# Aidan900/ppa-nbody-collisions

Hardware: AMD Instinct MI355X
Metric: body-pair-interactions/sec at N=262144 (higher is better)
Workload: dtype f32; 1 GPU; BASELINE.json configs[3] (the metric's configuration): N=262144 bodies, fp32, radii 0, reference initial condition (seed 1024), literal reference step semantics, 98 steps; bodies_after=262110, parallelism=single GPU

## Files before the change

ppa-nbody-collisions_amd/csrc/nbody_kernels.hpp:

```cpp
#pragma once
#include <hip/hip_runtime.h>
#include <stdint.h>
#include <type_traits>

#include "nbody.h"
#include "nbody_partition.h"

#pragma clang fp contract(off)

namespace nbk {

constexpr int kTile = 128;
constexpr int kWave = 64;

template <typename T> struct Rec;
template <> struct alignas(16) Rec<float> { float x, y, m, r; };
template <> struct alignas(32) Rec<double> { double x, y, m, r; };
template <typename T> struct alignas(2 * sizeof(T)) Vec2 { T x, y; };

struct alignas(16) RecPadded {
    double x, y, m, r, pad0, pad1;
    __device__ __forceinline__ RecPadded& operator=(const Rec<double>& o) { x = o.x; y = o.y; m = o.m; r = o.r; return *this; }
    __device__ __forceinline__ operator Rec<double>() const { return Rec<double>{x, y, m, r}; }
};
// ... 474 lines not shown
    __shared__ RecPadded tile_all[2][2][2 * kTile];                                                          \
    __shared__ int tile_bad_all[2][2][kTile / kWave];                                                        \
    __shared__ int tile_rnz_all[2][2][kTile / kWave];                                                        \
    RecPadded(&tile)[2][2 * kTile] = tile_all[threadIdx.x / kTile];                                          \
    int(&tile_bad)[2][kTile / kWave] = tile_bad_all[threadIdx.x / kTile];                                    \
    int(&tile_rnz)[2][kTile / kWave] = tile_rnz_all[threadIdx.x / kTile];
#define NB_V3_LANE const int lane = threadIdx.x % kTile;
#define NB_V3_WG const int wg = blockIdx.x * 2 + threadIdx.x / kTile;
#define NB_V3_BATCH 8
#define NB_V3_CONSTANTS constexpr int K = 1;
#define NB_V3_RANGE const int N = meta->n, lo = meta->lo, cnt = meta->cnt, step = meta->step;
#define NB_V3_REC(j) J[j]
#define NB_V3_VEL(i) Vown[i - lo]
#define NB_V3_PUT(q, i, out, vout) S_J[q] = out; S_V[q] = vout;
#define NB_V3_KEEP(q, i, a, v) S_J[q] = Rec<T>{a.xi, a.yi, a.mi, a.ri}; S_V[q] = v;
#define NB_V3_COUNT(pairs)                                                                                   \
    for (int sh = kWave / 2; sh > 0; sh >>= 1) pairs += __shfl_down(pairs, sh, kWave);                      \
    if ((lane & (kWave - 1)) == 0 && pairs) atomicAdd(&ctr->pairs, pairs);
#include "nbody_forces_v3.inc"
#undef NB_V3_ROTATE_PRIORITY
#undef NB_V3_TILE_REC
#undef NB_V3_REAL
#undef NB_V3_SIGNATURE
#undef NB_V3_LDS
#undef NB_V3_LANE
#undef NB_V3_WG
#undef NB_V3_BATCH
#undef NB_V3_CONSTANTS
#undef NB_V3_RANGE
#undef NB_V3_REC
#undef NB_V3_VEL
#undef NB_V3_PUT
#undef NB_V3_KEEP
#undef NB_V3_COUNT

#ifndef NBK_TEMPLATES_ONLY
#define NB_V3_REAL float
#define NB_V3_SIGNATURE                                                                                      \
    __global__ __launch_bounds__(2 * kTile, 4) void ref_layout_forces_v3_f32(                                \
        void* bodyData, float* __restrict__ updM, float* __restrict__ updR, const int N, StepParams<float> p)
#define NB_V3_LDS                                                                                            \
    __shared__ Rec<T> tile_all[2][2][2 * kTile];                                                             \
    __shared__ int tile_bad_all[2][2][kTile / kWave];                                                        \
    __shared__ int tile_rnz_all[2][2][kTile / kWave];                                                        \
    Rec<T>(&tile)[2][2 * kTile] = tile_all[threadIdx.x / kTile];                                             \
    int(&tile_bad)[2][kTile / kWave] = tile_bad_all[threadIdx.x / kTile];                                    \
    int(&tile_rnz)[2][kTile / kWave] = tile_rnz_all[threadIdx.x / kTile];
#define NB_V3_LANE const int lane = threadIdx.x % kTile;
#define NB_V3_WG const int wg = blockIdx.x * 2 + threadIdx.x / kTile;
#define NB_V3_BATCH 8
#define NB_V3_CONSTANTS                                                                                      \
    constexpr int K = 1;                                                                                     \
    constexpr bool kLog = false;
#define NB_V3_RANGE                                                                                          \
    constexpr int lo = 0, step = 0, ev_cap = 0;                                                              \
    const int cnt = N;                                                                                       \
    Event* const ev = nullptr;                                                                               \
    Counters* const ctr = nullptr;                                                                           \
    const Vec2<float>* __restrict__ P = reinterpret_cast<const Vec2<float>*>(bodyData);        \
    Vec2<float>* __restrict__ V = reinterpret_cast<Vec2<float>*>(bodyData) + N;                              \
    const float* __restrict__ M = reinterpret_cast<const float*>(V + N);                                     \
    const float* __restrict__ R = M + N;
#define NB_V3_REC(j) Rec<float>{P[j].x, P[j].y, M[j], R[j]}
#define NB_V3_VEL(i) V[i]
#define NB_V3_PUT(q, i, out, vout) (void)q; updM[i] = out.m; updR[i] = out.r; V[i] = vout;
#define NB_V3_KEEP(q, i, a, v) (void)q;
#define NB_V3_COUNT(pairs) (void)pairs;
#include "nbody_forces_v3.inc"
#undef NB_V3_REAL
#undef NB_V3_SIGNATURE
#undef NB_V3_LDS
#undef NB_V3_LANE
#undef NB_V3_WG
#undef NB_V3_BATCH
#undef NB_V3_CONSTANTS
#undef NB_V3_RANGE
#undef NB_V3_REC
#undef NB_V3_VEL
#undef NB_V3_PUT
#undef NB_V3_KEEP
#undef NB_V3_COUNT
#endif

typedef __attribute__((address_space(3))) void* LdsPtr;
typedef int Int4 __attribute__((ext_vector_type(4)));
typedef float Float2 __attribute__((ext_vector_type(2)));
typedef float Float4 __attribute__((ext_vector_type(4)));
typedef volatile __attribute__((address_space(3))) Int4* LdsInt4Ptr;
typedef volatile __attribute__((address_space(3))) Float4* LdsFloat4Ptr;

constexpr int kRingDeadSeq = 0x40000000;
constexpr unsigned long long kIndexError = 1ull << 32;
__device__ __forceinline__ int batch_checked_count(int n, int stride) { return (n < 0 || n > stride) ? -1 : n; }

#pragma clang diagnostic push
#pragma clang diagnostic ignored "-Winline-asm"
__device__ __forceinline__ void load_to_lds_b32(const void* base, unsigned byte_offset, unsigned lds_dst) {
    asm volatile("s_mov_b32 m0, %0\n\ts_nop 0\n\tglobal_load_lds_dword %1, %2"
                 ::"s"(lds_dst), "v"(byte_offset), "s"(base) : "memory", "m0");
}
#pragma clang diagnostic pop
__device__ __forceinline__ unsigned lds_offset_of(const void* p) { return (unsigned)(unsigned long long)(LdsPtr)p; }

struct RingArgs {
    const Vec2<float>* Vown;
    Rec<float>* S_J;
    Vec2<float>* S_V;
    const Meta* meta;
    StepParams<float> p;
    Event* ev;
    int ev_cap;
    Counters* ctr;
    const float* tile_rmax;
    const float* Jt;
    int cap_own;
    int n_tiles;
    unsigned* q_head;
    unsigned long long* q_done;
    unsigned long long* q_state;
    unsigned q_launch;
    int q_rings;
    int q_whole;
    int q_seg_tiles;
};
typedef __attribute__((address_space(1))) unsigned* GlobalU32Ptr;
typedef __attribute__((address_space(1))) unsigned long long* GlobalU64Ptr;
typedef volatile __attribute__((address_space(3))) long long* LdsI64Ptr;
template <typename A>
__device__ __forceinline__ A ring_late_arg(unsigned byte_offset) {
#if defined(__HIP_DEVICE_COMPILE__)
    typedef const __attribute__((address_space(4))) char* KernargBytes;
    const KernargBytes ka = (KernargBytes)__builtin_amdgcn_kernarg_segment_ptr();
    asm volatile("" : "+s"(byte_offset));
    return *(const __attribute__((address_space(4))) A*)(ka + byte_offset);
#else
    (void)byte_offset;
    return A{};
#endif
}
#define NB_RING_LATE(field) \
    ring_late_arg<decltype(((const RingArgs*)nullptr)->field)>((unsigned)__builtin_offsetof(RingArgs, field))

template <bool kLog, int kW, int kT, int kSleep, bool kProbe, int kRings, bool kQueue = false>
__global__ __launch_bounds__(kRings * kW * kWave) __attribute__((amdgpu_waves_per_eu(4, 4)))
void forces_ring_f32(const RingArgs args) {
    typedef float T;
    const Meta* __restrict__ const meta = args.meta;
    const float* __restrict__ const tile_rmax = args.tile_rmax;
    const float* __restrict__ const Jt = args.Jt;
    typedef Pair<float>::type V2;
    static_assert(kTile % kT == 0 && kT % 8 == 0 && kT <= kWave, "turn length");
    constexpr int kTurnsPerTile = kTile / kT;
    constexpr bool kSolo = kW == 1;
    static_assert(kSolo || kW % kTurnsPerTile == 0, "a wave's successive turns are whole tiles apart");
    constexpr int kTilesPerRound = kW / kTurnsPerTile;
    constexpr int kWin = kWave + kT;
    static_assert(kSolo ? kRings == 16 && !kProbe : kRings == 1 || kRings == 2 || kRings == 4, "rings (64 bodies each) per workgroup");
    static_assert(!kQueue || kSolo || kW == kTurnsPerTile, "persistent form: an item is whole tiles and a wave keeps its part of every tile");
    __shared__ float win_all[kRings][kW][2][4][kWin];
    __shared__ Int4 hand_all[kSolo ? 1 : kRings][kWave];
    __shared__ Float4 hand_m_all[kRings][kWave];
    __shared__ int solo_done_all[kSolo ? kRings : 1];
    __shared__ long long item_all[kQueue && !kSolo ? kRings : 1][2];
    const int N = meta->n, lo = meta->lo, cnt = meta->cnt;
    const bool all_bounded = (meta->summary & kSummaryUnbounded) == 0, any_radius = (meta->summary & kSummaryRadius) != 0;
    const bool nan_screen = meta->summary == 0;
    const int tid = threadIdx.x;
    const int wv = __builtin_amdgcn_readfirstlane(tid / kWave);
    const int ring = wv / kW;
    const int w = wv % kW;
    const int l = tid % kWave;
    const int wg = blockIdx.x;
    const int slot = wg * kRings + ring;
    float(&win)[kW][2][4][kWin] = win_all[ring];
    Int4(&hand)[kWave] = hand_all[kSolo ? 0 : ring];
    Float4(&hand_m)[kWave] = hand_m_all[ring];
    const int nb = N < kTile ? 1 : N / kTile;
    const bool lit = args.p.literal != 0;
    const int ntiles = lit ? nb : (N + kTile - 1) / kTile;
    const int nturns = ntiles * kTurnsPerTile;
    const int q_spin_limit = kQueue ? __builtin_amdgcn_readfirstlane(args.p.spin_limit) : 0;
    bool dead = false;
    int timeouts = 0;
    unsigned long long pr_eval = 0, pr_wait = 0, pr_chain = 0, pr_check = 0, pr_polls = 0, pr_turns = 0, pr_t0 = 0, pr_r0 = 0;
    int seq_base = 0;
    int claims = 0;
    Int4 solo_h = Int4{0, 0, 0, 0};
    typedef volatile __attribute__((address_space(3))) int* LdsIntPtr;
    int solo_done = 0;
    if (kSolo) *(LdsIntPtr)&solo_done_all[wv] = 0;
    if (kQueue && !kSolo) {
        if (w == 0) {
            *(LdsInt4Ptr)&hand[l] = Int4{0, 0, 0, 0};
            if (l < 2) *(LdsI64Ptr)&item_all[ring][l] = 0ll;
        }
        __syncthreads();
        if (kProbe) { pr_t0 = __builtin_readcyclecounter(); pr_r0 = wall_clock64(); }
    }
    for (;;) {
        int ring_g = slot;
        int tau_lo = 0, tau_hi = nturns, seg = 0;
        if (kQueue) {
            const LdsI64Ptr entry = (LdsI64Ptr)&item_all[ring][claims & 1];
            claims += 1;
            const int q_whole = NB_RING_LATE(q_whole), q_cut = NB_RING_LATE(q_rings) - q_whole;
            const int seg_tiles = NB_RING_LATE(q_seg_tiles);
            const int nseg = (ntiles + seg_tiles - 1) / seg_tiles;
            auto decode = [&](int k) -> int {
                if ((long long)k >= q_whole + (long long)q_cut * nseg) return 0;
                ring_g = k; seg = 0; tau_lo = 0; tau_hi = nturns;
                if (k >= q_whole) {
                    seg = (k - q_whole) / q_cut;
                    ring_g = q_whole + (k - q_whole) % q_cut;
                    tau_lo = seg * seg_tiles * kTurnsPerTile;
                    tau_hi = tau_lo + seg_tiles * kTurnsPerTile < nturns ? tau_lo + seg_tiles * kTurnsPerTile : nturns;
                }
                const long long first = (long long)(lo / kTile + ring_g / 2) * kTile + (ring_g % 2) * kWave;
                return first >= (long long)lo + cnt ? 1 : 2;
            };
            auto decode_solo = [&](int k) -> int {
                const int rings = q_whole + q_cut;
                const int lead = q_whole < ntiles ? q_whole : ntiles;
                const int solo_nseg = 1 + (ntiles - lead + seg_tiles - 1) / seg_tiles;
                if ((long long)k >= (long long)rings * solo_nseg) return 0;
                seg = k / rings;
                ring_g = k - seg * rings;
                tau_lo = seg == 0 ? 0 : (lead + (seg - 1) * seg_tiles) * kTurnsPerTile;
                tau_hi = seg == 0 ? lead * kTurnsPerTile : tau_lo + seg_tiles * kTurnsPerTile;
                tau_hi = tau_hi < nturns ? tau_hi : nturns;
                const long long first = (long long)(lo / kTile + ring_g / 2) * kTile + (ring_g % 2) * kWave;
                return first >= (long long)lo + cnt ? 1 : 2;
            };
            int k = 0x7fffffff, what = 0;
            if (w == 0) {
                do {
                    unsigned drawn = 0;
                    if (l == 0) drawn = __hip_atomic_fetch_add((GlobalU32Ptr)NB_RING_LATE(q_head), 1u, __ATOMIC_RELAXED, __HIP_MEMORY_SCOPE_AGENT);
                    k = __builtin_amdgcn_readfirstlane((int)(drawn < 0x7fffffffu ? drawn : 0x7fffffffu));
                    what = kSolo ? decode_solo(k) : decode(k);
                } while (what == 1);
                if (!kSolo && l == 0) *entry = ((long long)claims << 32) | (long long)k;
            } else {
                for (int spins = 0;;) {
                    const long long e = *entry;
                    if (__builtin_amdgcn_readfirstlane((int)(e >> 32)) == claims) { k = __builtin_amdgcn_readfirstlane((int)e); break; }
                    if (++spins > q_spin_limit) { timeouts += 1; break; }
                    if (kSleep > 0) __builtin_amdgcn_s_sleep(kSleep);
                }
                what = decode(k);
            }
            if (what != 2) break;
        }
        const int half = ring_g % 2;
        const int b = lo / kTile + ring_g / 2;
        const int t0 = half * kWave;
        const int t = t0 + l;
        const long long blk0 = (long long)b * kTile;

        const bool mine = blk0 + t >= lo && blk0 + t < (long long)lo + cnt;
        const bool active = mine && blk0 + t < N && (!lit || blk0 + t < (long long)nb * kTile);
        auto body_index64 = [&]() -> long long {
            int lane = l;
            asm volatile("" : "+v"(lane));
            return blk0 + t0 + lane;
        };
        T xi = 0, yi = 0, ri = 0;
        {
            T mi = 0;
            if (mine) {
                const long long i64 = blk0 + t;
                const int i = (int)(i64 < 0x7fffffff ? i64 : 0x7fffffff);
                const float* me = Jt + (size_t)(i / kTile) * (4 * kTile) + (i % kTile);
                xi = me[0]; yi = me[kTile]; mi = me[2 * kTile]; ri = me[3 * kTile];
            }
            asm volatile("" : "+v"(xi), "+v"(yi), "+v"(mi), "+v"(ri));
            if (kQueue) {
                if (w == 0) {
                    Int4 h0 = Int4{0, 0, kSolo ? 0 : seq_base, 0};
                    Float4 m0 = Float4{mi, ri, mi, 0.0f};
                    bool late = false;
                    for (int spins = 0; !kSolo;) {
                        const Int4 h = *(LdsInt4Ptr)&hand[l];
                        if (__ballot(h.z < seq_base) == 0ull) break;
                        if (++spins > q_spin_limit) { late = true; break; }
                        if (kSleep > 0) __builtin_amdgcn_s_sleep(kSleep);
                    }
                    if (tau_lo > 0) {
                        const GlobalU64Ptr done = (GlobalU64Ptr)NB_RING_LATE(q_done) + ring_g;
                        const unsigned long long want = ((unsigned long long)NB_RING_LATE(q_launch) << 32) | (unsigned)seg;
                        for (int spins = 0; !late;) {
                            const unsigned long long have = __hip_atomic_load(done, __ATOMIC_RELAXED, __HIP_MEMORY_SCOPE_AGENT);
                            if (__ballot(have < want) == 0ull) break;
                            if (++spins > q_spin_limit) { late = true; break; }
                            if (kSleep > 0) __builtin_amdgcn_s_sleep(kSleep);
                        }
                        const GlobalU64Ptr rs = (GlobalU64Ptr)NB_RING_LATE(q_state) + (size_t)ring_g * (4 * kWave) + l;
                        const unsigned long long s0 = __hip_atomic_load(rs, __ATOMIC_RELAXED, __HIP_MEMORY_SCOPE_AGENT);
                        const unsigned long long s1 = __hip_atomic_load(rs + kWave, __ATOMIC_RELAXED, __HIP_MEMORY_SCOPE_AGENT);
                        const unsigned long long s2 = __hip_atomic_load(rs + 2 * kWave, __ATOMIC_RELAXED, __HIP_MEMORY_SCOPE_AGENT);
                        const unsigned long long s3 = __hip_atomic_load(rs + 3 * kWave, __ATOMIC_RELAXED, __HIP_MEMORY_SCOPE_AGENT);
                        h0 = Int4{(int)(unsigned)s0, (int)(unsigned)(s0 >> 32),
                                  (int)(unsigned)s1 >= kRingDeadSeq ? kRingDeadSeq : kSolo ? 0 : seq_base, (int)(unsigned)(s1 >> 32)};
                        m0 = Float4{__uint_as_float((unsigned)s2), __uint_as_float((unsigned)(s2 >> 32)), __uint_as_float((unsigned)s3), 0.0f};
                    }
                    if (late) { timeouts += 1; dead = true; }
                    if (kSolo && __ballot(h0.z >= kRingDeadSeq) != 0ull) dead = true;
                    if (dead) {
                        h0 = Int4{(int)0x7fc00000, (int)0x7fc00000, kRingDeadSeq, 0};
                        m0.x = m0.y = __builtin_nanf("");
                    }
                    *(LdsFloat4Ptr)&hand_m[l] = m0;
                    if (kSolo) solo_h = h0;
                    else *(LdsInt4Ptr)&hand[l] = h0;
                }
            } else if (w == 0) {
                if (kSolo) solo_h = Int4{0, 0, 0, 0};
                else *(LdsInt4Ptr)&hand[l] = Int4{0, 0, 0, 0};
                *(LdsFloat4Ptr)&hand_m[l] = Float4{mi, ri, mi, 0.0f};
            }
        }
        const int spin_limit = __builtin_amdgcn_readfirstlane(args.p.spin_limit);
        const bool lane_ok = !active || ((abs_(xi) < kCoordBound) && (abs_(yi) < kCoordBound));
        const bool wave_ok = __ballot(!lane_ok) == 0ull;
        int pairs_rare = 0;
        const LdsInt4Ptr hand_l = (LdsInt4Ptr)&hand[l];
        const LdsFloat4Ptr hand_m_l = (LdsFloat4Ptr)&hand_m[l];
        if (!kQueue) {
            if (!kSolo) __syncthreads();
            if (blk0 + t0 >= (long long)lo + cnt) return;
        }
        typedef const volatile __attribute__((address_space(3))) int* LdsSeqPtr;
        auto seq_of_ring_of = [&](int lane) -> LdsSeqPtr { return (LdsSeqPtr)&hand_all[lane % kRings][0] + 2; };
        LdsSeqPtr seq_look_kept = seq_of_ring_of(kLog ? 0 : l);
        if (!kLog && !kSolo && kRings > 1) asm volatile("" : "+v"(seq_look_kept));
        auto any_ring_ahead = [&]() -> bool {
            if (kLog) {
                int ahead = *seq_of_ring_of(ring + 1);
                if (kRings == 4) {
                    const int o2 = *seq_of_ring_of(ring + 2), o3 = *seq_of_ring_of(ring + 3);
                    ahead = ahead > o2 ? ahead : o2;
                    ahead = ahead > o3 ? ahead : o3;
                }
                return *seq_of_ring_of(ring) < ahead;
            }
            const int theirs = *seq_look_kept;
            const int ours = ((LdsSeqPtr)hand_l)[2];
            return __ballot(ours < theirs) != 0ull;
        };
        if (kProbe && !kQueue) { pr_t0 = __builtin_readcyclecounter(); pr_r0 = wall_clock64(); }

        auto tile_start_slow = [&](int kk) -> long long {
            if (!lit) return (long long)kk * kTile;
            return (blk0 % N + (long long)kk * kTile) % N;
        };
        typedef typename std::conditional<kLog, long long, unsigned>::type Idx;
        const Idx Nu = (Idx)N;
        auto round_on = [&](Idx st) -> Idx {
            st += kTilesPerRound * kTile;
            if (lit) while (st >= Nu) st -= Nu;
            return st;
        };
        auto tile_on = [&](Idx st) -> Idx {
            st += kTile;
            if (lit) while (st >= Nu) st -= Nu;
            return st;
        };
        auto tile_len = [&](int kk, Idx st) -> int {
            if (lit) return (kk == nb - 1) ? N % (kTile + 1) : kTile;
            if (kLog) return (Nu - st) < kTile ? (int)(Nu - st) : kTile;
            const int rest = (int)(Nu - st);
            return rest < kTile ? rest : kTile;
        };
        auto turn_kind = [&](int tau, Idx st) -> int {
            if (tau >= tau_hi) return 0;
            return tile_len(tau / kTurnsPerTile, st) == kTile ? 1 : 2;
        };
        auto fast_tile = [&](int kk) -> bool { return lit || kk != b; };
        const int wbase0 = lit ? t0 : 0;
        const int nwin = lit ? (kWave + kT - 1) : kT;
        auto entry_bytes_of = [&](int lane) -> unsigned {
            return ((unsigned)(wbase0 + (w % kTurnsPerTile) * kT + lane) & (kTile - 1)) * (unsigned)sizeof(T);
        };
        unsigned entry0_kept = kLog ? 0u : entry_bytes_of(l);
        if (!kLog) asm volatile("" : "+v"(entry0_kept));
        auto window_offset = [&](Idx st, unsigned e) -> unsigned {
            const unsigned src = (unsigned)st + e;
            const unsigned wrapped = src - (unsigned)N;
            const unsigned idx = src < wrapped ? src : wrapped;
            return ((idx / kTile) * (4u * kTile) + (idx % kTile)) * (unsigned)sizeof(T);
        };
        auto issue_entries = [&](unsigned tile_byte, unsigned byte_offset, unsigned base, unsigned comp_bytes) {
            unsigned long long plane = kTile * sizeof(T);
            asm volatile("" : "+s"(plane));
            if (kLog) {
                const unsigned long long last = (unsigned long long)tile_byte + byte_offset + 3 * kTile * sizeof(T) + sizeof(T);
                if (last > (unsigned long long)NB_RING_LATE(n_tiles) * (4 * kTile * sizeof(T))) {
                    atomicAdd(&NB_RING_LATE(ctr)->errors, kIndexError);
                    return;
                }
            }
            const char* const src = (const char*)Jt + tile_byte;
            load_to_lds_b32(src, byte_offset, base);
            load_to_lds_b32(src + plane, byte_offset, base + comp_bytes);
            load_to_lds_b32(src + 2 * plane, byte_offset, base + 2 * comp_bytes);
            if (any_radius) load_to_lds_b32(src + 3 * plane, byte_offset, base + 3 * comp_bytes);
        };
        auto solo_quarter = [&](int tau) -> unsigned { return (unsigned)(tau % kTurnsPerTile) * (kT * (unsigned)sizeof(T)); };
        auto issue_window = [&](Idx st, int buf, unsigned quarter_bytes) {
            const unsigned base = __builtin_amdgcn_readfirstlane(lds_offset_of(&win[w][buf][0][0]));
            if (kLog) {
                int lane = l;
                asm volatile("" : "+v"(lane));
                const unsigned e0 = (unsigned)(wbase0 + (w % kTurnsPerTile) * kT + lane + (kSolo ? quarter_bytes / (unsigned)sizeof(T) : 0u)) & (kTile - 1);
                const unsigned e1 = e0 ^ kWave;
                if (((unsigned)st & (kTile - 1)) == 0u && st + kTile <= Nu) {
                    const unsigned tile_byte = ((unsigned)st / kTile) * (4u * kTile * (unsigned)sizeof(T));
                    if (l < nwin) issue_entries(tile_byte, e0 * (unsigned)sizeof(T), base, kWin * (unsigned)sizeof(T));
                    if (l + kWave < nwin) issue_entries(tile_byte, e1 * (unsigned)sizeof(T), base + kWave * (unsigned)sizeof(T), kWin * (unsigned)sizeof(T));
                } else {
                    if (l < nwin) issue_entries(0u, window_offset(st, e0), base, kWin * (unsigned)sizeof(T));
                    if (l + kWave < nwin) issue_entries(0u, window_offset(st, e1), base + kWave * (unsigned)sizeof(T), kWin * (unsigned)sizeof(T));
                }
                return;
            }
            const unsigned entry0_bytes = kSolo ? (entry0_kept + quarter_bytes) & (kTile * (unsigned)sizeof(T) - 1u) : entry0_kept;
            const unsigned entry1_bytes = entry0_bytes ^ (kWave * (unsigned)sizeof(T));
            if (((unsigned)st & (kTile - 1)) == 0u && st + kTile <= Nu) {
                const unsigned tile_byte = ((unsigned)st / kTile) * (4u * kTile * (unsigned)sizeof(T));
                if (l < nwin) issue_entries(tile_byte, entry0_bytes, base, kWin * (unsigned)sizeof(T));
                if (l + kWave < nwin) issue_entries(tile_byte, entry1_bytes, base + kWave * (unsigned)sizeof(T), kWin * (unsigned)sizeof(T));
            } else {
                if (l < nwin) issue_entries(0u, window_offset(st, entry0_bytes / (unsigned)sizeof(T)), base, kWin * (unsigned)sizeof(T));
                if (l + kWave < nwin) issue_entries(0u, window_offset(st, entry1_bytes / (unsigned)sizeof(T)), base + kWave * (unsigned)sizeof(T), kWin * (unsigned)sizeof(T));
            }
        };
        static_assert(2 * kWin >= kTile, "a whole tile fits the two window buffers");
        float* const whole = &win[w][0][0][0];
        auto issue_truncated = [&](Idx st, int L) {
            const unsigned base = __builtin_amdgcn_readfirstlane(lds_offset_of(whole));
            if (l < L) issue_entries(0u, window_offset(st, (unsigned)l), base, kTile * (unsigned)sizeof(T));
            if (l + kWave < L) issue_entries(0u, window_offset(st, (unsigned)(l + kWave)), base + kWave * (unsigned)sizeof(T), kTile * (unsigned)sizeof(T));
        };
        auto window_record = [&](const float* comp0, int stride, int idx) -> Rec<T> {
            return Rec<T>{comp0[idx], comp0[stride + idx], comp0[2 * stride + idx], any_radius ? comp0[3 * stride + idx] : 0.0f};
        };
        auto window_rmax = [&](Idx st) -> float {
            if (!any_radius) return 0.0f;
            const int ta = __builtin_amdgcn_readfirstlane((int)(st / kTile));
            if (kLog && (ta < 0 || ta + 1 >= NB_RING_LATE(n_tiles))) {
                if (l == 0) atomicAdd(&NB_RING_LATE(ctr)->errors, kIndexError);
                return __builtin_inff();
            }
            const float ra = tile_rmax[ta], rb = tile_rmax[ta + 1];
            const float rw = (st + kTile > Nu) ? tile_rmax[0] : 0.0f;
            const float rab = ra > rb ? ra : rb;
            return rab > rw ? rab : rw;
        };
        struct WindowState { bool fast; float rmax; };
        auto check_window = [&](int kind, int kk, int buf, Idx st_w) -> WindowState {
            if (kind != 1) return WindowState{false, 0.0f};
            asm volatile("s_waitcnt vmcnt(0)" ::: "memory");
            __builtin_amdgcn_wave_barrier();
            if (all_bounded) return WindowState{wave_ok && fast_tile(kk), window_rmax(st_w)};
            Rec<T> r0{0, 0, 0, 0}, r1{0, 0, 0, 0};
            if (l < nwin) r0 = window_record(&win[w][buf][0][0], kWin, l);
            if (l + kWave < nwin) r1 = window_record(&win[w][buf][0][0], kWin, l + kWave);
            const bool bad0 = !((abs_(r0.x) < kCoordBound) && (abs_(r0.y) < kCoordBound));
            const bool bad1 = !((abs_(r1.x) < kCoordBound) && (abs_(r1.y) < kCoordBound));
            WindowState ws;
            ws.fast = __ballot(bad0 || bad1) == 0ull && wave_ok && fast_tile(kk);
            ws.rmax = window_rmax(st_w);
            return ws;
        };
        auto general_turn = [&](BodyAcc<T>& a, int kind, int kk, long long st, int L, int off0, int buf, bool bounded) {
            const long long i64 = body_index64();
            const int i = (int)(i64 < 0x7fffffff ? i64 : 0x7fffffff);
            const T growth = NB_RING_LATE(p.growth);
            Event* const ev = kLog ? NB_RING_LATE(ev) : nullptr;
            const int ev_cap = kLog ? NB_RING_LATE(ev_cap) : 0;
            Counters* const ctr = kLog ? NB_RING_LATE(ctr) : nullptr;
            const int step = kLog ? meta->step : 0;
            if (kind == 2) {
                asm volatile("s_waitcnt vmcnt(0)" ::: "memory");
                __builtin_amdgcn_wave_barrier();
            }
            const int hi = off0 + kT < L ? off0 + kT : L;
            int lane_entry = lit ? l : 0;
            asm volatile("" : "+v"(lane_entry));
            const int t = (int)(i64 - blk0);
    #pragma unroll 1
            for (int off = off0; off < hi; ++off) {
                int sidx;
                long long j;
                if (lit) {
                    if (kk == 0 && off == 0) continue;
                    sidx = (L == kTile) ? ((t + off) & (kTile - 1)) : ((t + off) % L);
                    j = st + sidx;
                    if (j >= N) j %= N;
                } else {
                    sidx = off;
                    j = st + off;
                    if (j == i64) continue;
                }
                const Rec<T> rec = kind == 1 ? window_record(&win[w][buf][0][0], kWin, lane_entry + (off - off0))
                                             : window_record(whole, kTile, sidx);
                if (bounded) {
                    const T dx = rec.x - a.xi, dy = rec.y - a.yi;
                    const T d2 = (dx * dx) + (dy * dy);
                    const T rs = a.ri + rec.r;
                    if (!(d2 <= fma_(rs, rs, kFastLo))) {
                        const T inv = fast_chain(d2).inv;
                        a.fx = a.fx + (dx * rec.m) * inv;
                        a.fy = a.fy + (dy * rec.m) * inv;
                        continue;
                    }
                }
                interact<T, kLog>(a, rec, growth, i, (int)j, ev, ev_cap, ctr, step);
            }
        };

        const int tau0 = tau_lo + w;
        const int dseq = kQueue ? seq_base - tau_lo : 0;
        Idx st = (Idx)tile_start_slow(tau0 / kTurnsPerTile);
        int buf = 0;
        int plain_turns = 0;
        bool first_plain = false;
        int kind = turn_kind(tau0, st);
        if (kind == 1) issue_window(st, buf, solo_quarter(tau0));
        if (kind == 2) issue_truncated(st, tile_len(tau0 / kTurnsPerTile, st));
        WindowState cur = check_window(kind, tau0 / kTurnsPerTile, buf, st);
        for (int tau = tau0; tau < tau_hi; tau += kW) {
            unsigned long long pt0 = 0, pt1 = 0, pt2 = 0, pt3 = 0;
            if (kProbe) pt0 = __builtin_readcyclecounter();
            const int kk = tau / kTurnsPerTile;
            const int off0 = (tau % kTurnsPerTile) * kT;
            const int L = tile_len(kk, st);
            const bool fast = cur.fast;
            const Idx st_next = kSolo ? ((tau + 1) % kTurnsPerTile == 0 ? tile_on(st) : st) : round_on(st);
            const int kind_next = turn_kind(tau + kW, st_next);
            if (kind_next == 1) issue_window(st_next, buf ^ 1, solo_quarter(tau + kW));
            const bool first = lit && tau == 0;
            if (kSolo) {
                solo_done += 1;
                *(LdsIntPtr)&solo_done_all[wv] = solo_done;
                const int theirs = *(LdsIntPtr)&solo_done_all[l % kRings];
                if (__ballot(solo_done < theirs) != 0ull) __builtin_amdgcn_s_setprio(1);
                else __builtin_amdgcn_s_setprio(0);
            }
            if (!kSolo && kRings > 1) {
                if (any_ring_ahead()) __builtin_amdgcn_s_setprio(1);
                else __builtin_amdgcn_s_setprio(0);
            }
            V2 termx[kT / 2], termy[kT / 2];
            auto term_x = [&](int r) -> float { return (r & 1) ? termx[r / 2].y : termx[r / 2].x; };
            auto term_y = [&](int r) -> float { return (r & 1) ? termy[r / 2].y : termy[r / 2].x; };
            unsigned long long flag = 0;
            auto evaluate = [&](auto screen_tag) {
                constexpr bool kScreen = decltype(screen_tag)::value;
                const float* wx = &win[w][buf][0][lit ? l : 0];
                const float* wy = wx + kWin;
                const float* wm = wx + 2 * kWin;
                const V2 ownx = {xi, xi}, owny = {yi, yi};
                const float reach = abs_(ri) + cur.rmax;
                const float threshold = __builtin_fmaf(reach, reach, kFastLo);
                float closest = kFastHi;
                V2 pxa = {wx[0], wx[1]}, pxb = {wx[2], wx[3]}, pya = {wy[0], wy[1]}, pyb = {wy[2], wy[3]};
                V2 pma = {wm[0], wm[1]}, pmb = {wm[2], wm[3]};
    #pragma unroll
                for (int r0 = 0; r0 < kT; r0 += 4) {
                    const V2 xa = pxa, xb = pxb, ya = pya, yb = pyb, ma = pma, mb = pmb;
                    if (r0 + 4 < kT) {
                        pxa = V2{wx[r0 + 4], wx[r0 + 5]}; pxb = V2{wx[r0 + 6], wx[r0 + 7]};
                        pya = V2{wy[r0 + 4], wy[r0 + 5]}; pyb = V2{wy[r0 + 6], wy[r0 + 7]};
                        pma = V2{wm[r0 + 4], wm[r0 + 5]}; pmb = V2{wm[r0 + 6], wm[r0 + 7]};
                    }
                    __builtin_amdgcn_sched_barrier(0);
                    const V2 dxa = xa - ownx, dxb = xb - ownx;
                    const V2 dya = ya - owny, dyb = yb - owny;
                    const V2 sxa = dxa * dxa, sxb = dxb * dxb;
                    const V2 sya = dya * dya, syb = dyb * dyb;
                    const V2 d2a = sxa + sya, d2b = sxb + syb;
                    if (kScreen) {
                        const float first_d2 = (r0 == 0 && first) ? kFastHi : d2a.x;
                        asm("v_min3_f32 %0, %1, %2, %3" : "=v"(closest) : "v"(closest), "v"(first_d2), "v"(d2a.y));
                        asm("v_min3_f32 %0, %1, %2, %3" : "=v"(closest) : "v"(closest), "v"(d2b.x), "v"(d2b.y));
                    }
                    V2 inva, invb;
                    fast_inv_cube2x2(d2a, d2b, inva, invb);
                    const V2 txa = dxa * ma, txb = dxb * mb;
                    const V2 tya = dya * ma, tyb = dyb * mb;
                    termx[r0 / 2] = txa * inva; termx[r0 / 2 + 1] = txb * invb;
                    termy[r0 / 2] = tya * inva; termy[r0 / 2 + 1] = tyb * invb;
                    asm volatile("" : "+v"(termx[r0 / 2]), "+v"(termx[r0 / 2 + 1]), "+v"(termy[r0 / 2]), "+v"(termy[r0 / 2 + 1]));
                }
                if (kScreen) flag = le_mask(closest, threshold);
                if (first) { termx[0].x = 0.0f; termy[0].x = 0.0f; }
            };
            if (fast) {
                if (nan_screen) evaluate(std::false_type{});
                else evaluate(std::true_type{});
            }
            if (kProbe) pt1 = __builtin_readcyclecounter();
            Int4 h = Int4{0, 0, 0, 0};
            bool timed_out = false;
            if (!kSolo) __builtin_amdgcn_s_setprio(3);
            const int sq = kSolo ? 0 : tau + dseq;
            if (kSolo) h = solo_h;
            if (!kSolo && (kQueue || tau > 0)) {
                int spins = 0;
                for (;;) {
                    h = *hand_l;
                    if (__ballot(h.z < sq) == 0ull) break;
                    if (++spins > spin_limit) { timed_out = true; break; }
                    if (kSleep > 0) __builtin_amdgcn_s_sleep(kSleep);
                }
                if (kProbe) pr_polls += spins + 1;
            }
            if (kProbe) pt2 = __builtin_readcyclecounter();
            bool plain = fast && flag == 0ull && !dead && !timed_out && (kSolo || __ballot(h.z != sq) == 0ull);
            if (__builtin_expect(plain, 1)) {
                float fx = __int_as_float(h.x), fy = __int_as_float(h.y);
    #pragma unroll
                for (int r = 0; r < kT; ++r) {
                    fx = fx + term_x(r);
                    asm("" : "+v"(fx));
                    fy = fy + term_y(r);
                }
                if (nan_screen) flag = __builtin_amdgcn_fcmpf(fx, fy, 8 );
                if (__builtin_expect(flag == 0ull, 1)) {
                    if (kSolo) solo_h = Int4{(int)__float_as_uint(fx), (int)__float_as_uint(fy), 0, h.w};
                    else *hand_l = Int4{(int)__float_as_uint(fx), (int)__float_as_uint(fy), sq + 1, h.w};
                    if (!kSolo) __builtin_amdgcn_s_setprio(0);
                    plain_turns += 1;
                    first_plain = first_plain || first;
                } else {
                    plain = false;
                }
            }
            if (__builtin_expect(!plain, 0)) {
                BodyAcc<T> a;
                a.xi = xi; a.yi = yi; a.ri = ri;
                a.fx = __int_as_float(h.x); a.fy = __int_as_float(h.y);
                a.deleted = h.w & 1;
                const Float4 hm = *hand_m_l;
                a.mnew = hm.x; a.rnew = hm.y; a.mi = hm.z;
                timeouts += timed_out ? 1 : 0;
                dead = dead || timed_out || __ballot(h.z >= kRingDeadSeq) != 0ull;
                const unsigned m_before = __float_as_uint(a.mnew), r_before = __float_as_uint(a.rnew);
                if (fast && nan_screen) {
    #pragma unroll
                    for (int r = 0; r < kT; ++r) flag |= __builtin_amdgcn_fcmpf(term_x(r), term_y(r), 8);
                }
                if (fast) {
                    unsigned hits = 0;
                    bool odd = false;
                    unsigned long long todo = flag & __ballot(active);
                    while (todo != 0ull) {
                        const int fl = __builtin_amdgcn_readfirstlane((int)__builtin_ctzll(todo));
                        todo &= todo - 1ull;
                        const T xf = __int_as_float(__builtin_amdgcn_readlane((int)__float_as_uint(a.xi), fl));
                        const T yf = __int_as_float(__builtin_amdgcn_readlane((int)__float_as_uint(a.yi), fl));
                        const T mf = __int_as_float(__builtin_amdgcn_readlane((int)__float_as_uint(a.mi), fl));
                        const T rf = __int_as_float(__builtin_amdgcn_readlane((int)__float_as_uint(a.ri), fl));
                        int r = l & (kT - 1);
                        asm volatile("" : "+v"(r));
                        const Rec<T> rec = window_record(&win[w][buf][0][0], kWin, (lit ? fl : 0) + r);
                        const T dx = rec.x - xf, dy = rec.y - yf;
                        const T d2 = (dx * dx) + (dy * dy);
                        const T rs = rf + rec.r;
                        const bool is_pair = l < kT && !(first && r == 0);
                        const bool hit = d2 <= rs * rs && (mf >= rec.m || mf < rec.m);
                        const bool guarded = d2 <= fma_(rs, rs, kFastLo);
                        const unsigned long long hm = __ballot(is_pair && hit);
                        const unsigned long long om = __ballot(is_pair && guarded && !hit);
                        if (l == fl) { hits = (unsigned)hm; odd = om != 0ull; }
                    }
                    if (active) {
                        if (odd) {
                            general_turn(a, 1, kk, st, L, off0, buf, true);
                        } else {
                            float fx = a.fx, fy = a.fy;
    #pragma unroll
                            for (int r = 0; r < kT; ++r) {
                                const float nx = add_unmerged(fx, term_x(r));
                                const float ny = add_unmerged(fy, term_y(r));
                                const bool skip = ((hits >> r) & 1u) != 0u;
                                fx = skip ? fx : nx;
                                fy = skip ? fy : ny;
                            }
                            a.fx = fx; a.fy = fy;
                            unsigned rest = hits;
                            int lane_entry = lit ? l : 0;
                            asm volatile("" : "+v"(lane_entry));
                            const T growth = NB_RING_LATE(p.growth);
                            while (rest != 0u) {
                                const int r = __builtin_ctz(rest);
                                rest &= rest - 1u;
                                const Rec<T> rec = window_record(&win[w][buf][0][0], kWin, lane_entry + r);
                                const bool ge = a.mi >= rec.m;
                                if (ge) {
                                    a.mnew = a.mnew + rec.m;
                                    a.rnew = a.rnew + rec.r * growth;
                                } else {
                                    a.deleted = 1;
                                }
                                if (kLog) {
                                    const long long i64 = body_index64();
                                    const int i = (int)(i64 < 0x7fffffff ? i64 : 0x7fffffff);
                                    long long j = lit ? (long long)st + (((int)(i64 - blk0) + off0 + r) & (kTile - 1)) : (long long)st + off0 + r;
                                    if (j >= N) j %= N;
                                    Counters* const ctr = NB_RING_LATE(ctr);
                                    const unsigned long long slot = atomicAdd(&ctr->events, 1ull);
                                    if (slot < (unsigned long long)NB_RING_LATE(ev_cap))
                                        NB_RING_LATE(ev)[slot] = Event{meta->step, i, (int)j, ge ? 0 : 1};
                                }
                            }
                        }
                        pairs_rare += kT - (first ? 1 : 0);
                    }
                } else if (active) {
                    general_turn(a, kind, kk, st, L, off0, buf, false);
                    const int hi = off0 + kT < L ? off0 + kT : L;
                    if (lit) {
                        if (hi > off0) pairs_rare += (hi - off0) - ((kk == 0 && off0 == 0) ? 1 : 0);
                    } else {
                        const long long i64 = body_index64();
                        for (int off = off0; off < hi; ++off) pairs_rare += ((long long)st + off != i64) ? 1 : 0;
                    }
                }
                if (dead) {
                    a.fx = a.fy = a.mnew = a.rnew = __builtin_nanf("");
                    a.deleted = 0;
                }
                if (__float_as_uint(a.mnew) != m_before || __float_as_uint(a.rnew) != r_before)
                    *hand_m_l = Float4{a.mnew, a.rnew, a.mi, 0.0f};
                if (kSolo) solo_h = Int4{(int)__float_as_uint(a.fx), (int)__float_as_uint(a.fy), dead ? kRingDeadSeq : 0, a.deleted & 1};
                else *hand_l = Int4{(int)__float_as_uint(a.fx), (int)__float_as_uint(a.fy), dead ? kRingDeadSeq : sq + 1,
                                    a.deleted & 1};
                if (!kSolo) __builtin_amdgcn_s_setprio(0);
            }
            if (kProbe) pt3 = __builtin_readcyclecounter();
            if (kind_next == 2) issue_truncated(st_next, tile_len((tau + kW) / kTurnsPerTile, st_next));
            buf ^= 1;
            st = st_next;
            kind = kind_next;
            cur = check_window(kind, (tau + kW) / kTurnsPerTile, buf, st);
            if (kProbe) {
                pr_eval += pt1 - pt0; pr_wait += pt2 - pt1; pr_chain += pt3 - pt2;
                pr_check += __builtin_readcyclecounter() - pt3;
            }
        }
        if ((kQueue || mine) && (tau_hi - 1) % kW == w) {
            const Int4 hf = kSolo ? solo_h : *hand_l;
            const Float4 hm = *hand_m_l;
            if (kQueue && tau_hi < nturns) {
                const GlobalU64Ptr rs = (GlobalU64Ptr)NB_RING_LATE(q_state) + (size_t)ring_g * (4 * kWave) + l;
                __hip_atomic_store(rs, ((unsigned long long)(unsigned)hf.y << 32) | (unsigned)hf.x, __ATOMIC_RELAXED, __HIP_MEMORY_SCOPE_AGENT);
                __hip_atomic_store(rs + kWave, ((unsigned long long)(unsigned)hf.w << 32) | (unsigned)hf.z, __ATOMIC_RELAXED, __HIP_MEMORY_SCOPE_AGENT);
                __hip_atomic_store(rs + 2 * kWave, ((unsigned long long)__float_as_uint(hm.y) << 32) | __float_as_uint(hm.x), __ATOMIC_RELAXED, __HIP_MEMORY_SCOPE_AGENT);
                __hip_atomic_store(rs + 3 * kWave, (unsigned long long)__float_as_uint(hm.z), __ATOMIC_RELAXED, __HIP_MEMORY_SCOPE_AGENT);
                asm volatile("s_waitcnt vmcnt(0)" ::: "memory");
                if (l == 0)
                    __hip_atomic_store((GlobalU64Ptr)NB_RING_LATE(q_done) + ring_g,
                                       ((unsigned long long)NB_RING_LATE(q_launch) << 32) | (unsigned)(seg + 1),
                                       __ATOMIC_RELAXED, __HIP_MEMORY_SCOPE_AGENT);
            } else if (mine) {
                const long long i64 = body_index64();
                const int q = (int)(i64 - lo);
                BodyAcc<T> a;
                a.xi = xi; a.yi = yi; a.ri = ri; a.mi = hm.z;
                a.fx = __int_as_float(hf.x); a.fy = __int_as_float(hf.y);
                a.mnew = hm.x; a.rnew = hm.y; a.deleted = hf.w & 1;
                Rec<T>* const S_J = NB_RING_LATE(S_J);
                Vec2<T>* const S_V = NB_RING_LATE(S_V);
                const bool q_ok = q >= 0 && q < NB_RING_LATE(cap_own);
                const Vec2<T> v = q_ok ? NB_RING_LATE(Vown)[q] : Vec2<T>{0, 0};
                if (!q_ok) {
                    atomicAdd(&NB_RING_LATE(ctr)->errors, kIndexError);
                } else if (active) {
                    const StepParams<T> p = NB_RING_LATE(p);
                    Rec<T> out; Vec2<T> vout;
                    finish_body<T>(a, v, p, out, vout);
                    S_J[q] = out;
                    S_V[q] = vout;
                } else {
                    S_J[q] = Rec<T>{a.xi, a.yi, a.mi, a.ri};
                    S_V[q] = v;
                }
            }
            if (kQueue && !kSolo) *hand_l = Int4{hf.x, hf.y, hf.z >= kRingDeadSeq ? kRingDeadSeq : seq_base + (tau_hi - tau_lo) + 1, hf.w};
        }
        {
            unsigned long long pairs = 0;
            if (active) pairs = (unsigned long long)((long long)plain_turns * kT - (first_plain ? 1 : 0) + pairs_rare);
            for (int sh = kWave / 2; sh > 0; sh >>= 1) pairs += __shfl_down(pairs, sh, kWave);
            if (l == 0 && pairs) atomicAdd(&NB_RING_LATE(ctr)->pairs, pairs);
        }
        if (kProbe) pr_turns += (unsigned long long)((tau_hi - tau0 + kW - 1) / kW);
        if (!kQueue) break;
        seq_base += tau_hi - tau_lo + 1;
    }
    Counters* const ctr = NB_RING_LATE(ctr);
    if (kSolo) *(LdsIntPtr)&solo_done_all[wv] = 0;
    if (kQueue && w == 0 && l == 0) {
        const GlobalU32Ptr head = (GlobalU32Ptr)NB_RING_LATE(q_head);
        if (__hip_atomic_fetch_add(head + 1, 1u, __ATOMIC_RELAXED, __HIP_MEMORY_SCOPE_AGENT) == gridDim.x * kRings - 1u) {
            __hip_atomic_store(head, 0u, __ATOMIC_RELAXED, __HIP_MEMORY_SCOPE_AGENT);
            __hip_atomic_store(head + 1, 0u, __ATOMIC_RELAXED, __HIP_MEMORY_SCOPE_AGENT);
        }
    }
    if (timeouts != 0 && l == 0) atomicAdd(&ctr->errors, (unsigned long long)timeouts);
    if (kProbe && l == 0) {
        Event* const ev = NB_RING_LATE(ev);
        const int ev_cap = NB_RING_LATE(ev_cap);
        atomicAdd(&ctr->probe[0], pr_eval); atomicAdd(&ctr->probe[1], pr_wait);
        atomicAdd(&ctr->probe[2], pr_chain); atomicAdd(&ctr->probe[3], pr_check);
        atomicAdd(&ctr->probe[4], pr_polls);
        atomicAdd(&ctr->probe[5], pr_turns);
        if (wg == 0 && w == 0) {
            ctr->probe[6] = __builtin_readcyclecounter() - pr_t0;
            ctr->probe[7] = wall_clock64() - pr_r0;
        }
        if (w == 0) {
            const unsigned long long at = atomicAdd(&ctr->events, 1ull);
            if (at < (unsigned long long)ev_cap)
                ev[at] = Event{(int)(unsigned)pr_r0, (int)(unsigned)wall_clock64(),
                               (int)__builtin_amdgcn_s_getreg((31 << 11) | 4),
                               (int)((__builtin_amdgcn_s_getreg((31 << 11) | 20) << 20) | (unsigned)slot)};
        }
    }
}

constexpr int kCompactBlock = 1024;
template <typename T>
__device__ __forceinline__ void store_tiled(float* __restrict__ Jt, int i, const Rec<T>& r) {
    float* t = Jt + (size_t)(i / kTile) * (4 * kTile) + (i % kTile);
    t[0] = (float)r.x; t[kTile] = (float)r.y; t[2 * kTile] = (float)r.m; t[3 * kTile] = (float)r.r;
}
#ifndef NBK_TEMPLATES_ONLY
__global__ __launch_bounds__(256) void records_to_tiles_f32(const Rec<float>* __restrict__ J, int n, float* __restrict__ Jt) {
    const int i = blockIdx.x * 256 + threadIdx.x;
    if (i < n) store_tiled(Jt, i, J[i]);
}
#endif

template <typename T>
__device__ __forceinline__ bool compact_keep(T mass) { return mass != (T)0; }

template <int B>
__device__ __forceinline__ int compact_block_count(bool keep) {
    __shared__ int wsum[B / kWave];
    const unsigned long long bal = __ballot(keep);
    if ((threadIdx.x & (kWave - 1)) == 0) wsum[threadIdx.x / kWave] = __popcll(bal);
    __syncthreads();
    int s = 0;
    if (threadIdx.x == 0)
        for (int w = 0; w < B / kWave; ++w) s += wsum[w];
    return s;
}

struct CompactOffset { int off, below, here; };
template <int B>
__device__ __forceinline__ CompactOffset compact_offset(bool keep, const int* __restrict__ lower_counts) {
    static_assert(B / kWave >= 2, "red[] carries the two totals");
    __shared__ int wsum[B / kWave];
    __shared__ int red[B / kWave];
    const int lane = threadIdx.x & (kWave - 1);
    const int wid = threadIdx.x / kWave;
    int part = 0;
    for (int bidx = threadIdx.x; bidx < (int)blockIdx.x; bidx += B) part += lower_counts[bidx];
    for (int sh = kWave / 2; sh > 0; sh >>= 1) part += __shfl_down(part, sh, kWave);
    if (lane == 0) red[wid] = part;
    const unsigned long long bal = __ballot(keep);
    if (lane == 0) wsum[wid] = __popcll(bal);
    __syncthreads();
    if (threadIdx.x == 0) {
        int s = 0, t = 0;
        for (int w = 0; w < B / kWave; ++w) s += red[w];
        for (int w = 0; w < B / kWave; ++w) t += wsum[w];
        red[0] = s;
        red[1] = t;
    }
    __syncthreads();
    const int below = red[0], here = red[1];
    int off = below;
    for (int w = 0; w < wid; ++w) off += wsum[w];
    off += __popcll(bal & ((1ull << lane) - 1ull));
    return CompactOffset{off, below, here};
}

template <typename T>
__global__ __launch_bounds__(kCompactBlock) void compact_count(const Rec<T>* __restrict__ S_J,
                                                               const Meta* __restrict__ meta,
                                                               int* __restrict__ blk_counts,
                                                               unsigned* __restrict__ tile_rmax, int n_tiles) {
    const int cnt = meta->cnt;
    const int q = blockIdx.x * kCompactBlock + threadIdx.x;
    if (q == 0) const_cast<Meta*>(meta)->summary = 0;
    for (int k = q; k < n_tiles; k += gridDim.x * kCompactBlock) tile_rmax[k] = 0u;
    const int s = compact_block_count<kCompactBlock>(q < cnt && compact_keep(S_J[q].m));
    if (threadIdx.x == 0) blk_counts[blockIdx.x] = s;
}

template <typename T>
__global__ __launch_bounds__(kCompactBlock) void compact_scatter(const Rec<T>* __restrict__ S_J,
                                                                 const Vec2<T>* __restrict__ S_V,
                                                                 const Meta* __restrict__ meta,
                                                                 const int* __restrict__ blk_counts, int nblk,
                                                                 SlotHeader* __restrict__ slot_hdr,
                                                                 Rec<T>* __restrict__ slot_recs,
                                                                 Vec2<T>* __restrict__ slot_vels) {
    const int cnt = meta->cnt;
    const int q = blockIdx.x * kCompactBlock + threadIdx.x;
    Rec<T> rec{};
    Vec2<T> vel{};
    bool keep = false;
    if (q < cnt) {
        rec = S_J[q];
        vel = S_V[q];
        keep = compact_keep(rec.m);
    }
    const CompactOffset o = compact_offset<kCompactBlock>(keep, blk_counts);
    if (threadIdx.x == 0 && (int)blockIdx.x == nblk - 1) {
        slot_hdr->count = o.below + o.here;
        slot_hdr->layout = (int)(reinterpret_cast<const Rec<T>*>(slot_vels) - slot_recs);
    }
    if (keep) {
        slot_recs[o.off] = rec;
        slot_vels[o.off] = vel;
    }
}

template <typename T>
__global__ __launch_bounds__(256) void unpack_slots(const unsigned char* __restrict__ gather, size_t slot_bytes,
                                                    int cap_own, int world, int rank, Rec<T>* __restrict__ J,
                                                    Vec2<T>* __restrict__ Vown, Meta* __restrict__ meta,
                                                    unsigned* __restrict__ tile_rmax, float* __restrict__ Jt,
                                                    Counters* __restrict__ ctr) {
    const int g = blockIdx.y;
    int off = 0, total = 0;
    bool bad_header = false;
    auto count_of = [&](int h) -> int {
        const SlotHeader* hd = reinterpret_cast<const SlotHeader*>(gather + (size_t)h * slot_bytes);
        const int c = hd->count;
        if (c < 0 || c > cap_own || hd->layout != cap_own) { bad_header = true; return c < 0 ? 0 : (c > cap_own ? cap_own : c); }
        return c;
    };
    for (int h = 0; h < world; ++h) {
        const int c = count_of(h);
        if (h < g) off += c;
        total += c;
    }
    if (bad_header && g == 0 && blockIdx.x == 0 && threadIdx.x == 0) atomicAdd(&ctr->errors, kIndexError);
    int lo, cnt;
    nbody_own_range_of(total, rank, world, &lo, &cnt);
// ... 312 lines not shown
```

Baseline: 2432 billion body-pair-interactions/sec.

## Trim solo-wave ring kernel state, window addressing, sync and pair counting

For the solo (one wave per ring) non-logging variant, the hand state is split into separate scalar-friendly registers and per-lane window entry offsets are precomputed, so per-turn address math drops out. The window radius max becomes wave-uniform through readfirstlane. The cross-ring progress handshake in LDS now runs only once per tile instead of every turn. Pair counts are accumulated per slot from a ballot popcount and flushed with one atomic at the end, replacing the per-item shuffle reduction. This cuts VALU and register pressure in the hot loop, at the cost of more specialised code paths and looser synchronisation between rings.

```diff
diff --git a/ppa-nbody-collisions_amd/csrc/nbody_kernels.hpp b/ppa-nbody-collisions_amd/csrc/nbody_kernels.hpp
--- a/ppa-nbody-collisions_amd/csrc/nbody_kernels.hpp
+++ b/ppa-nbody-collisions_amd/csrc/nbody_kernels.hpp
@@ -650,6 +650,7 @@
     static_assert(kTile % kT == 0 && kT % 8 == 0 && kT <= kWave, "turn length");
     constexpr int kTurnsPerTile = kTile / kT;
     constexpr bool kSolo = kW == 1;
+    constexpr bool kTrim = kSolo && !kLog;
     static_assert(kSolo || kW % kTurnsPerTile == 0, "a wave's successive turns are whole tiles apart");
     constexpr int kTilesPerRound = kW / kTurnsPerTile;
     constexpr int kWin = kWave + kT;
@@ -684,6 +685,9 @@
     int seq_base = 0;
     int claims = 0;
     Int4 solo_h = Int4{0, 0, 0, 0};
+    float solo_fx = 0.0f, solo_fy = 0.0f;
+    int solo_del = 0;
+    unsigned long long pairs_slot = 0;
     typedef volatile __attribute__((address_space(3))) int* LdsIntPtr;
     int solo_done = 0;
     if (kSolo) *(LdsIntPtr)&solo_done_all[wv] = 0;
@@ -808,11 +812,13 @@
                         m0.x = m0.y = __builtin_nanf("");
                     }
                     *(LdsFloat4Ptr)&hand_m[l] = m0;
-                    if (kSolo) solo_h = h0;
+                    if (kTrim) { solo_fx = __int_as_float(h0.x); solo_fy = __int_as_float(h0.y); solo_del = h0.w; }
+                    else if (kSolo) solo_h = h0;
                     else *(LdsInt4Ptr)&hand[l] = h0;
                 }
             } else if (w == 0) {
-                if (kSolo) solo_h = Int4{0, 0, 0, 0};
+                if (kTrim) { solo_fx = solo_fy = 0.0f; solo_del = 0; }
+                else if (kSolo) solo_h = Int4{0, 0, 0, 0};
                 else *(LdsInt4Ptr)&hand[l] = Int4{0, 0, 0, 0};
                 *(LdsFloat4Ptr)&hand_m[l] = Float4{mi, ri, mi, 0.0f};
             }
@@ -879,8 +885,12 @@
         auto entry_bytes_of = [&](int lane) -> unsigned {
             return ((unsigned)(wbase0 + (w % kTurnsPerTile) * kT + lane) & (kTile - 1)) * (unsigned)sizeof(T);
         };
-        unsigned entry0_kept = kLog ? 0u : entry_bytes_of(l);
-        if (!kLog) asm volatile("" : "+v"(entry0_kept));
+        unsigned entry0_kept = kLog || kTrim ? 0u : entry_bytes_of(l);
+        if (!kLog && !kTrim) asm volatile("" : "+v"(entry0_kept));
+        static_assert(!kTrim || (kT == 32 && kWave == 64 && kTile == 128), "the quarter is 128 bytes, the lanes' offsets 256");
+        unsigned entry_lane_kept = kTrim ? (unsigned)l * (unsigned)sizeof(T) : 0u;
+        unsigned entry_wrap_kept = kTrim ? ((unsigned)l * (unsigned)sizeof(T) + 384u) & 511u : 0u;
+        if (kTrim) asm volatile("" : "+v"(entry_lane_kept), "+v"(entry_wrap_kept));
         auto window_offset = [&](Idx st, unsigned e) -> unsigned {
             const unsigned src = (unsigned)st + e;
             const unsigned wrapped = src - (unsigned)N;
@@ -921,6 +931,25 @@
                 }
                 return;
             }
+            if (kTrim) {
+                const unsigned h0 = ((quarter_bytes >> 7) + ((unsigned)wbase0 >> 5)) & 3u, h1 = h0 ^ 2u;
+                if (((unsigned)st & (kTile - 1)) == 0u && st + kTile <= Nu) {
+                    const unsigned tile_byte = ((unsigned)st / kTile) * (4u * kTile * (unsigned)sizeof(T));
+                    if (l < nwin) {
+                        if (h0 == 3u) issue_entries(tile_byte, entry_wrap_kept, base, kWin * (unsigned)sizeof(T));
+                        else issue_entries(tile_byte + (h0 << 7), entry_lane_kept, base, kWin * (unsigned)sizeof(T));
+                    }
+                    if (l + kWave < nwin) {
+                        if (h1 == 3u) issue_entries(tile_byte, entry_wrap_kept, base + kWave * (unsigned)sizeof(T), kWin * (unsigned)sizeof(T));
+                        else issue_entries(tile_byte + (h1 << 7), entry_lane_kept, base + kWave * (unsigned)sizeof(T), kWin * (unsigned)sizeof(T));
+                    }
+                } else {
+                    const unsigned e0 = ((entry_lane_kept + (h0 << 7)) & 511u) / (unsigned)sizeof(T), e1 = e0 ^ kWave;
+                    if (l < nwin) issue_entries(0u, window_offset(st, e0), base, kWin * (unsigned)sizeof(T));
+                    if (l + kWave < nwin) issue_entries(0u, window_offset(st, e1), base + kWave * (unsigned)sizeof(T), kWin * (unsigned)sizeof(T));
+                }
+                return;
+            }
             const unsigned entry0_bytes = kSolo ? (entry0_kept + quarter_bytes) & (kTile * (unsigned)sizeof(T) - 1u) : entry0_kept;
             const unsigned entry1_bytes = entry0_bytes ^ (kWave * (unsigned)sizeof(T));
             if (((unsigned)st & (kTile - 1)) == 0u && st + kTile <= Nu) {
@@ -954,12 +983,16 @@
             const float rab = ra > rb ? ra : rb;
             return rab > rw ? rab : rw;
         };
+        auto window_rmax_scalar = [&](Idx st) -> float {
+            if (!any_radius) return 0.0f;
+            return __uint_as_float((unsigned)__builtin_amdgcn_readfirstlane((int)__float_as_uint(window_rmax(st))));
+        };
         struct WindowState { bool fast; float rmax; };
         auto check_window = [&](int kind, int kk, int buf, Idx st_w) -> WindowState {
             if (kind != 1) return WindowState{false, 0.0f};
             asm volatile("s_waitcnt vmcnt(0)" ::: "memory");
             __builtin_amdgcn_wave_barrier();
-            if (all_bounded) return WindowState{wave_ok && fast_tile(kk), window_rmax(st_w)};
+            if (all_bounded) return WindowState{wave_ok && fast_tile(kk), kTrim ? window_rmax_scalar(st_w) : window_rmax(st_w)};
             Rec<T> r0{0, 0, 0, 0}, r1{0, 0, 0, 0};
             if (l < nwin) r0 = window_record(&win[w][buf][0][0], kWin, l);
             if (l + kWave < nwin) r1 = window_record(&win[w][buf][0][0], kWin, l + kWave);
@@ -967,7 +1000,7 @@
             const bool bad1 = !((abs_(r1.x) < kCoordBound) && (abs_(r1.y) < kCoordBound));
             WindowState ws;
             ws.fast = __ballot(bad0 || bad1) == 0ull && wave_ok && fast_tile(kk);
-            ws.rmax = window_rmax(st_w);
+            ws.rmax = kTrim ? window_rmax_scalar(st_w) : window_rmax(st_w);
             return ws;
         };
         auto general_turn = [&](BodyAcc<T>& a, int kind, int kk, long long st, int L, int off0, int buf, bool bounded) {
@@ -1038,7 +1071,7 @@
             const int kind_next = turn_kind(tau + kW, st_next);
             if (kind_next == 1) issue_window(st_next, buf ^ 1, solo_quarter(tau + kW));
             const bool first = lit && tau == 0;
-            if (kSolo) {
+            if (kSolo && (!kTrim || tau % kTurnsPerTile == 0)) {
                 solo_done += 1;
                 *(LdsIntPtr)&solo_done_all[wv] = solo_done;
                 const int theirs = *(LdsIntPtr)&solo_done_all[l % kRings];
@@ -1103,7 +1136,8 @@
             bool timed_out = false;
             if (!kSolo) __builtin_amdgcn_s_setprio(3);
             const int sq = kSolo ? 0 : tau + dseq;
-            if (kSolo) h = solo_h;
+            if (kTrim) h = Int4{(int)__float_as_uint(solo_fx), (int)__float_as_uint(solo_fy), dead ? kRingDeadSeq : 0, solo_del};
+            else if (kSolo) h = solo_h;
             if (!kSolo && (kQueue || tau > 0)) {
                 int spins = 0;
                 for (;;) {
@@ -1123,10 +1157,12 @@
                     fx = fx + term_x(r);
                     asm("" : "+v"(fx));
                     fy = fy + term_y(r);
+                    if (kTrim) asm("" : "+v"(fy));
                 }
                 if (nan_screen) flag = __builtin_amdgcn_fcmpf(fx, fy, 8 );
                 if (__builtin_expect(flag == 0ull, 1)) {
-                    if (kSolo) solo_h = Int4{(int)__float_as_uint(fx), (int)__float_as_uint(fy), 0, h.w};
+                    if (kTrim) { solo_fx = fx; solo_fy = fy; }
+                    else if (kSolo) solo_h = Int4{(int)__float_as_uint(fx), (int)__float_as_uint(fy), 0, h.w};
                     else *hand_l = Int4{(int)__float_as_uint(fx), (int)__float_as_uint(fy), sq + 1, h.w};
                     if (!kSolo) __builtin_amdgcn_s_setprio(0);
                     plain_turns += 1;
@@ -1232,7 +1268,8 @@
                 }
                 if (__float_as_uint(a.mnew) != m_before || __float_as_uint(a.rnew) != r_before)
                     *hand_m_l = Float4{a.mnew, a.rnew, a.mi, 0.0f};
-                if (kSolo) solo_h = Int4{(int)__float_as_uint(a.fx), (int)__float_as_uint(a.fy), dead ? kRingDeadSeq : 0, a.deleted & 1};
+                if (kTrim) { solo_fx = a.fx; solo_fy = a.fy; solo_del = a.deleted & 1; }
+                else if (kSolo) solo_h = Int4{(int)__float_as_uint(a.fx), (int)__float_as_uint(a.fy), dead ? kRingDeadSeq : 0, a.deleted & 1};
                 else *hand_l = Int4{(int)__float_as_uint(a.fx), (int)__float_as_uint(a.fy), dead ? kRingDeadSeq : sq + 1,
                                     a.deleted & 1};
                 if (!kSolo) __builtin_amdgcn_s_setprio(0);
@@ -1249,7 +1286,8 @@
             }
         }
         if ((kQueue || mine) && (tau_hi - 1) % kW == w) {
-            const Int4 hf = kSolo ? solo_h : *hand_l;
+            const Int4 hf = kTrim ? Int4{(int)__float_as_uint(solo_fx), (int)__float_as_uint(solo_fy), dead ? kRingDeadSeq : 0, solo_del}
+                          : kSolo ? solo_h : *hand_l;
             const Float4 hm = *hand_m_l;
             if (kQueue && tau_hi < nturns) {
                 const GlobalU64Ptr rs = (GlobalU64Ptr)NB_RING_LATE(q_state) + (size_t)ring_g * (4 * kWave) + l;
@@ -1288,7 +1326,16 @@
             }
             if (kQueue && !kSolo) *hand_l = Int4{hf.x, hf.y, hf.z >= kRingDeadSeq ? kRingDeadSeq : seq_base + (tau_hi - tau_lo) + 1, hf.w};
         }
-        {
+        if (kTrim) {
+            const long long lanes = (long long)__builtin_popcountll(__ballot(active));
+            pairs_slot += (unsigned long long)(lanes * ((long long)plain_turns * kT - (first_plain ? 1 : 0)));
+            if (__ballot(pairs_rare != 0) != 0ull) {
+                unsigned long long pairs = (unsigned long long)(long long)pairs_rare;
+                for (int sh = kWave / 2; sh > 0; sh >>= 1) pairs += __shfl_down(pairs, sh, kWave);
+                pairs_slot += ((unsigned long long)(unsigned)__builtin_amdgcn_readfirstlane((int)(unsigned)(pairs >> 32)) << 32) |
+                              (unsigned)__builtin_amdgcn_readfirstlane((int)(unsigned)pairs);
+            }
+        } else {
             unsigned long long pairs = 0;
             if (active) pairs = (unsigned long long)((long long)plain_turns * kT - (first_plain ? 1 : 0) + pairs_rare);
             for (int sh = kWave / 2; sh > 0; sh >>= 1) pairs += __shfl_down(pairs, sh, kWave);
@@ -1299,6 +1346,7 @@
         seq_base += tau_hi - tau_lo + 1;
     }
     Counters* const ctr = NB_RING_LATE(ctr);
+    if (kTrim && l == 0 && pairs_slot) atomicAdd(&ctr->pairs, pairs_slot);
     if (kSolo) *(LdsIntPtr)&solo_done_all[wv] = 0;
     if (kQueue && w == 0 && l == 0) {
         const GlobalU32Ptr head = (GlobalU32Ptr)NB_RING_LATE(q_head);
```

After: 2457 billion body-pair-interactions/sec, median of 6. +1.0%, better.
